# jdalcorso/radar-sounder-crw

Measured on AMD Instinct MI355X. Metric: radargram columns/sec (CRW fwd+bwd), higher is better.
Workload: dtype f32 (conv2-5 multiply on the bf16 matrix cores with hi/lo operand pairs, fp32 accumulate: fp32-grade; everything else fp32); 1 GPU; one synthetic 512x4096 radargram per GPU per step = 8 items [T=32,N=63,16x16] (patch 16x16, overlap (8, 0)), tau=0.01, CNN encoder, fwd+bwd+all-reduce+Adam; parallelism=dp1 (independent sequences), chain=fp32 MFMA 16x16x4, prefix form, encoder_convs=bf16x3

## Files before the change

radar-sounder-crw_amd/csrc/encoder_conv.hip:

```cpp
#include "crw_common.h"
#include <type_traits>
#include <cstdlib>

namespace crw {
namespace {

constexpr int IMG_W = 10, PAD_W = 12, NPIX = 100, NPAD = 144, MT = 7;

typedef __bf16 bf8 __attribute__((ext_vector_type(8)));
typedef short s4v __attribute__((ext_vector_type(4)));
typedef short s8v __attribute__((ext_vector_type(8)));
typedef __attribute__((address_space(3))) char *lds_cp;

__device__ inline uint16_t f2bf(float x) { return __builtin_bit_cast(uint16_t, (__bf16)x); }
__device__ inline float bf2f(uint16_t h) { return __builtin_bit_cast(float, (uint32_t)h << 16); }

template <int C>
constexpr int row_stride() { return C * 2 + 16; }
template <int C>
constexpr int plane_bytes() { return NPAD * row_stride<C>(); }
template <int C>
__device__ inline int px_off(int pp, int chunk) { return pp * row_stride<C>() + 16 * chunk; }
template <int C>
constexpr int crs() { return C * 2 + 32; }
// ... 485 lines not shown
  constexpr int NT = NCI / 16;
  constexpr int WCI = NT < 4 ? NT : 4, WCO = NW / WCI;
  constexpr int NCOW = NCO / 16 / WCO;
  static_assert(NT == WCI && COUT % NCO == 0 && CIN % NCI == 0, "tiling");
  constexpr int NGRP_CI = CIN / NCI;
  extern __shared__ __attribute__((aligned(16))) char lds[];
  char *xs = lds, *ys = lds + NPL * XPL;

  constexpr int NGRP = NGRP_CI * (COUT / NCO);
  const int wg_slice = a.xcd_map ? ((int)blockIdx.x / 8 / NGRP) * 8 + (int)blockIdx.x % 8 : (int)blockIdx.x / NGRP;
  const int wg_grp = a.xcd_map ? ((int)blockIdx.x / 8) % NGRP : (int)blockIdx.x % NGRP;
  const int grp_ci = wg_grp % NGRP_CI, grp_co = wg_grp / NGRP_CI;
  const int ci_base = grp_ci * NCI, co_base = grp_co * NCO;
  const int tid = threadIdx.x, lane = tid & 63, wave = tid >> 6, g = lane >> 4;
  const int wci = wave % WCI, wco = wave / WCI;
  const int co0w = wco * NCOW * 16;

  f32x4 acc[9][NCOW];
#pragma unroll
  for (int t = 0; t < 9; ++t)
#pragma unroll
    for (int j = 0; j < NCOW; ++j) acc[t][j] = f32x4{0.f, 0.f, 0.f, 0.f};
  f32x4 accb[NCOW];
#pragma unroll
  for (int j = 0; j < NCOW; ++j) accb[j] = f32x4{0.f, 0.f, 0.f, 0.f};
  const bool bias_wave = grp_ci == 0 && __builtin_amdgcn_readfirstlane(wci) == 0;

  const int p_begin = wg_slice * a.patches_per_block;
  const int p_end = min(a.P, p_begin + a.patches_per_block);
  const uint32_t xs_a = (uint32_t)(uintptr_t)(lds_cp)xs, ys_a = (uint32_t)(uintptr_t)(lds_cp)ys;

  for (int pl = 0; pl < NPL; ++pl) {
    zero_halo<NCI, NTH, XS>(xs + pl * XPL + XTAIL * XS, tid);
    for (int c = tid; c < XTAIL * XS / 16; c += NTH) *reinterpret_cast<uint4 *>(xs + pl * XPL + 16 * c) = uint4{0, 0, 0, 0};
    for (int c = tid; c < (1 + TAILPIX) * YS / 16; c += NTH) *reinterpret_cast<uint4 *>(ys + pl * YPL + NPIX * YS + 16 * c) = uint4{0, 0, 0, 0};
  }

  constexpr int XCH = NCI / 8, XTOT = NPIX * XCH, XIT = (XTOT + NTH - 1) / NTH;
  constexpr int YCH = NCO / 8, YTOT = NPIX * YCH, YIT = (YTOT + NTH - 1) / NTH;
  constexpr int TXC = XTAIL * XCH, TYC = TAILPIX * YCH, TTOT = NPL * (TXC + TYC), TIT = (TTOT + NTH - 1) / NTH;
#ifdef CRW_CONV_STAMPS
  long long ph_[4] = {0, 0, 0, 0}, prev_ = (long long)__builtin_amdgcn_s_memtime();
#define WG_STAMP(k) { const long long n_ = (long long)__builtin_amdgcn_s_memtime(); ph_[k] += n_ - prev_; prev_ = n_; }
#else
#define WG_STAMP(k)
#endif

  auto tail_src_dst = [&](int c, int &src, int &dst) {
    const int pl = c / (TXC + TYC), r = c % (TXC + TYC);
    if (r < TXC) {
      const int s = r / XCH, ch = r % XCH;
      dst = pl * XPL + s * XS + 16 * ch;
      src = pl * XPL + (XTAIL + 9 * PAD_W + s) * XS + 16 * ch;
    } else {
      const int q = r - TXC, j = q / YCH, ch = q % YCH;
      dst = NPL * XPL + pl * YPL + (YROWS + j) * YS + 16 * ch;
      src = NPL * XPL + pl * YPL + (NPIX - TAILPIX + j) * YS + 16 * ch;
    }
  };

  const int t16 = lane & 15, q4 = t16 >> 2, pq = t16 & 3;
  const uint32_t lane_col = 8 * (pq & 1) + 16 * (pq >> 1);
  auto row_addr = [&](int v, int carry, bool flush, uint32_t &ya, uint32_t &xa) {
    const int i = v - carry;
    int yrow = NPIX, xpix = XTAIL;
    if (v < carry) {
      const int t = NPIX - carry + v;
      yrow = YROWS + (t - (NPIX - TAILPIX));
      xpix = t - 90;
    } else if (!flush && i < NPIX) {
      yrow = i;
      xpix = XTAIL + (i / IMG_W) * PAD_W + (i % IMG_W);
    }
    ya = ys_a + yrow * YS + lane_col + 2 * co0w;
    xa = xs_a + xpix * XS + lane_col + 32 * wci;
  };
  auto kstep = [&](int ks, int carry, bool flush) {
    uint32_t ya_lo, ya_hi, xa_lo, xa_hi;
    row_addr(32 * ks + 4 * g + q4, carry, flush, ya_lo, xa_lo);
    row_addr(32 * ks + 4 * g + q4 + 16, carry, flush, ya_hi, xa_hi);
    bf8 ah[NCOW], al[NCOW];
    static_for<NCOW>([&](auto JC) {
      constexpr int j = decltype(JC)::value;
      ah[j] = tr_frag<32 * j>(ya_lo, ya_hi);
      if (SPLIT == 3) al[j] = tr_frag<YPL + 32 * j>(ya_lo, ya_hi);
    });
    bf8 bh[2], bl[2];
    auto read_b = [&](auto TC) {
      constexpr int tap = decltype(TC)::value;
      constexpr int XO = ((tap / 3) * PAD_W + (tap % 3)) * XS;
      bh[tap & 1] = tr_frag<XO>(xa_lo, xa_hi);
      if (SPLIT == 3) bl[tap & 1] = tr_frag<XPL + XO>(xa_lo, xa_hi);
    };
    read_b(std::integral_constant<int, 0>{});
    static_for<9>([&](auto TC) {
      constexpr int tap = decltype(TC)::value;
      if constexpr (tap < 8) {
        read_b(std::integral_constant<int, tap + 1>{});
        if (SPLIT == 3) asm volatile("s_waitcnt lgkmcnt(4)" ::: "memory");
        else asm volatile("s_waitcnt lgkmcnt(2)" ::: "memory");
      } else {
        asm volatile("s_waitcnt lgkmcnt(0)" ::: "memory");
      }
      __builtin_amdgcn_sched_barrier(0);
      if constexpr (tap == 0) {
        if (bias_wave) {
          const s8v o = {0x3f80, 0x3f80, 0x3f80, 0x3f80, 0x3f80, 0x3f80, 0x3f80, 0x3f80};
          const bf8 ones = __builtin_bit_cast(bf8, o);
#pragma unroll
          for (int j = 0; j < NCOW; ++j) {
            if (SPLIT == 3) accb[j] = __builtin_amdgcn_mfma_f32_16x16x32_bf16(al[j], ones, accb[j], 0, 0, 0);
            accb[j] = __builtin_amdgcn_mfma_f32_16x16x32_bf16(ah[j], ones, accb[j], 0, 0, 0);
          }
        }
      }
#pragma unroll
      for (int j = 0; j < NCOW; ++j) {
        if (SPLIT == 3) {
          acc[tap][j] = __builtin_amdgcn_mfma_f32_16x16x32_bf16(al[j], bh[tap & 1], acc[tap][j], 0, 0, 0);
          acc[tap][j] = __builtin_amdgcn_mfma_f32_16x16x32_bf16(ah[j], bl[tap & 1], acc[tap][j], 0, 0, 0);
        }
        acc[tap][j] = __builtin_amdgcn_mfma_f32_16x16x32_bf16(ah[j], bh[tap & 1], acc[tap][j], 0, 0, 0);
      }
    });
  };

  int carry = 0;
  uint4 tv[TIT];
#pragma unroll
  for (int i = 0; i < TIT; ++i) tv[i] = uint4{0, 0, 0, 0};
  if constexpr (MAP) {
    const int ntile = a.tiles_x * a.tiles_y;
    constexpr int WTOT = NPAD * XCH, WIT = (WTOT + NTH - 1) / NTH;
    for (int u = p_begin; u < p_end; ++u) {
      const int pq = u / ntile, tile = u % ntile;
      const int ty0 = (tile / a.tiles_x) * IMG_W, tx0 = (tile % a.tiles_x) * IMG_W;
      __syncthreads();
      for (int pl = 0; pl < NPL; ++pl) {
        uint4 xv[WIT];
        const uint16_t *src = (pl ? a.xl : a.xh) + ci_base;
#pragma unroll
        for (int i = 0; i < WIT; ++i) {
          const int c = min(tid + i * NTH, WTOT - 1), wp = c / XCH, ch = c % XCH;
          const int my = ty0 + wp / PAD_W - 1, mx = tx0 + wp % PAD_W - 1;
          const bool ok = my >= 0 && my < a.mh && mx >= 0 && mx < a.mw;
          const long off = (((long)pq * a.mh + min(max(my, 0), a.mh - 1)) * a.mw + min(max(mx, 0), a.mw - 1)) * CIN + 8 * ch;
          xv[i] = *reinterpret_cast<const uint4 *>(src + off);
          if (!ok) xv[i] = uint4{0, 0, 0, 0};
        }
#pragma unroll
        for (int i = 0; i < WIT; ++i) {
          const int c = tid + i * NTH;
          if (WTOT % NTH == 0 || c < WTOT) *reinterpret_cast<uint4 *>(xs + pl * XPL + (XTAIL + c / XCH) * XS + 16 * (c % XCH)) = xv[i];
        }
        uint4 yv[YIT];
        const uint16_t *ysrc = (pl ? a.dyl : a.dyh) + co_base;
#pragma unroll
        for (int i = 0; i < YIT; ++i) {
          const int c = min(tid + i * NTH, YTOT - 1), pix = c / YCH, ch = c % YCH;
          const int oy = ty0 + pix / IMG_W, ox = tx0 + pix % IMG_W;
          const bool ok = oy < a.mh && ox < a.mw;
          const long off = (((long)pq * a.mh + min(oy, a.mh - 1)) * a.mw + min(ox, a.mw - 1)) * COUT + 8 * ch;
          yv[i] = *reinterpret_cast<const uint4 *>(ysrc + off);
          if (!ok) yv[i] = uint4{0, 0, 0, 0};
        }
#pragma unroll
        for (int i = 0; i < YIT; ++i) {
          const int c = tid + i * NTH;
          if (YTOT % NTH == 0 || c < YTOT) *reinterpret_cast<uint4 *>(ys + pl * YPL + (c / YCH) * YS + 16 * (c % YCH)) = yv[i];
        }
      }
      __syncthreads();
#pragma unroll 1
      for (int ks = 0; ks < 4; ++ks) kstep(ks, 0, false);
    }
  }
  for (int p = MAP ? p_end : p_begin; p < p_end; ++p) {
    __syncthreads();
    WG_STAMP(3)
    {
#pragma unroll
      for (int i = 0; i < TIT; ++i) {
        const int c = tid + i * NTH;
        if (TTOT % NTH == 0 || c < TTOT) {
          int src, dst;
          tail_src_dst(c, src, dst);
          *reinterpret_cast<uint4 *>(xs + dst) = tv[i];
        }
      }
      uint4 xv[NPL][XIT], yv[NPL][YIT];
#pragma unroll
      for (int pl = 0; pl < NPL; ++pl) {
        const uint16_t *src = (pl ? a.xl : a.xh) + (long)p * NPIX * CIN + ci_base;
#pragma unroll
        for (int i = 0; i < XIT; ++i) {
          const int c = min(tid + i * NTH, XTOT - 1);
          xv[pl][i] = *reinterpret_cast<const uint4 *>(src + (long)(c / XCH) * CIN + 8 * (c % XCH));
        }
      }
#pragma unroll
      for (int pl = 0; pl < NPL; ++pl) {
        const uint16_t *src = ((pl && !a.dgap) ? a.dyl : a.dyh) + (long)p * NPIX * COUT + co_base;
#pragma unroll
        for (int i = 0; i < YIT; ++i) {
          const int c = min(tid + i * NTH, YTOT - 1);
          yv[pl][i] = *reinterpret_cast<const uint4 *>(src + (long)(c / YCH) * COUT + 8 * (c % YCH));
        }
      }
#pragma unroll
      for (int pl = 0; pl < NPL; ++pl)
#pragma unroll
        for (int i = 0; i < XIT; ++i) {
          const int c = tid + i * NTH;
          if (XTOT % NTH == 0 || c < XTOT)
            *reinterpret_cast<uint4 *>(xs + pl * XPL + (XTAIL + interior_pp(c / XCH)) * XS + 16 * (c % XCH)) = xv[pl][i];
        }
      if (a.dgap) {
        static_assert(NTH % YCH == 0, "a thread keeps its channel chunk");
        const int ch = tid % YCH;
        uint32_t gh[4], gl[4];
        gap_split8(a.dgap + (long)p * COUT + co_base + 8 * ch, gh, gl);
#pragma unroll
        for (int i = 0; i < YIT; ++i) {
          const int c = tid + i * NTH;
          if (YTOT % NTH == 0 || c < YTOT) {
            uint4 oh, ol;
            gap_mask8(yv[0][i], gh, gl, oh, ol);
            const int off = (c / YCH) * YS + 16 * ch;
            *reinterpret_cast<uint4 *>(ys + off) = oh;
            if (SPLIT == 3) *reinterpret_cast<uint4 *>(ys + YPL + off) = ol;
          }
        }
      } else {
#pragma unroll
        for (int pl = 0; pl < NPL; ++pl)
#pragma unroll
          for (int i = 0; i < YIT; ++i) {
            const int c = tid + i * NTH;
            if (YTOT % NTH == 0 || c < YTOT) *reinterpret_cast<uint4 *>(ys + pl * YPL + (c / YCH) * YS + 16 * (c % YCH)) = yv[pl][i];
          }
      }
    }
    __syncthreads();
    WG_STAMP(0)
    WG_STAMP(1)
#ifdef CRW_CONV_STAMPS
    if (a.stamps && tid == 0 && p - p_begin < 60)
      a.stamps[(long)blockIdx.x * 64 + 4 + (p - p_begin)] = (long long)__builtin_amdgcn_s_memtime();
#endif
    const int nks = carry == 8 ? 4 : 3;
#pragma unroll 1
    for (int ks = 0; ks < nks; ++ks) kstep(ks, carry, false);
    carry = carry == 8 ? 0 : carry + 4;
#pragma unroll
    for (int i = 0; i < TIT; ++i) {
      const int c = min(tid + i * NTH, TTOT - 1);
      int src, dst;
      tail_src_dst(c, src, dst);
      tv[i] = *reinterpret_cast<const uint4 *>(xs + src);
    }
    WG_STAMP(2)
  }
  if (carry > 0) {
    __syncthreads();
#pragma unroll
    for (int i = 0; i < TIT; ++i) {
      const int c = tid + i * NTH;
      if (TTOT % NTH == 0 || c < TTOT) {
        int src, dst;
        tail_src_dst(c, src, dst);
        *reinterpret_cast<uint4 *>(xs + dst) = tv[i];
      }
    }
    __syncthreads();
    kstep(0, carry, true);
  }
#ifdef CRW_CONV_STAMPS
  if (a.stamps && tid == 0)
    for (int k = 0; k < 4; ++k) a.stamps[(long)blockIdx.x * 64 + k] = ph_[k];
#endif

  float *dwp = a.dw_part + (long)wg_slice * COUT * CIN * 9;
#pragma unroll
  for (int tap = 0; tap < 9; ++tap)
#pragma unroll
    for (int j = 0; j < NCOW; ++j)
#pragma unroll
      for (int r = 0; r < 4; ++r) {
        const int co = co_base + co0w + 16 * j + 4 * g + r, ci = ci_base + 16 * wci + (lane & 15);
        dwp[((long)tap * COUT + co) * CIN + ci] = acc[tap][j][r];
      }
  if (bias_wave && (lane & 15) == 0) {
#pragma unroll
    for (int j = 0; j < NCOW; ++j)
#pragma unroll
      for (int r = 0; r < 4; ++r) a.db_part[(long)wg_slice * COUT + co_base + co0w + 16 * j + 4 * g + r] = accb[j][r];
  }
}

constexpr int W2_NCO = 128, W2_NCI = 64, W2_NW = 8, W2_KROWS = 32;
template <int C>
constexpr int w2_stride() { return 2 * C + 32; }

template <int SPLIT, int CIN, int COUT, int DIAG = 0>
__global__ __launch_bounds__(W2_NW * 64, 2) void conv3x3_wgrad2_kernel(WgradArgs a) {
  constexpr int NCO = W2_NCO, NCI = W2_NCI, NTH = W2_NW * 64, NPL = (SPLIT == 3) ? 2 : 1;
  constexpr int XS = w2_stride<NCI>(), XPL = NPAD * XS, XSLOT = NPL * XPL;
  constexpr int YS = w2_stride<NCO>(), YPL = W2_KROWS * YS, YSLOT = NPL * YPL;
  constexpr int NCOW = 4, WCI = 4;
  static_assert(COUT == NCO && CIN % NCI == 0, "tiling");
  constexpr int NGRP = CIN / NCI;
  extern __shared__ __attribute__((aligned(16))) char lds[];
  char *xs = lds, *ys = lds + 2 * XSLOT;
  char *gs = ys + 2 * YSLOT;

  const int wg_slice = a.xcd_map ? ((int)blockIdx.x / 8 / NGRP) * 8 + (int)blockIdx.x % 8 : (int)blockIdx.x / NGRP;
  const int grp_ci = a.xcd_map ? ((int)blockIdx.x / 8) % NGRP : (int)blockIdx.x % NGRP;
  const int ci_base = grp_ci * NCI;
  const int tid = threadIdx.x, lane = tid & 63, wave = tid >> 6, g = lane >> 4;
  const int wci = wave % WCI, wco = wave / WCI;
  const int wci_s = __builtin_amdgcn_readfirstlane(wci);
  const int co0w = wco * NCOW * 16;

  const int p_begin = wg_slice * a.patches_per_block;
  const int np = min(a.P, p_begin + a.patches_per_block) - p_begin;
  const int npx = np * NPIX;
  const int NK = (npx + W2_KROWS - 1) / W2_KROWS;

  f32x4 acc[9][NCOW];
#pragma unroll
  for (int t = 0; t < 9; ++t)
#pragma unroll
    for (int j = 0; j < NCOW; ++j) acc[t][j] = f32x4{0.f, 0.f, 0.f, 0.f};
  f32x4 accb = f32x4{0.f, 0.f, 0.f, 0.f};
  const bool bias_wg = grp_ci == 0;

  for (int c = tid; c < 2 * XSLOT / 16; c += NTH) *reinterpret_cast<uint4 *>(xs + 16 * c) = uint4{0, 0, 0, 0};

  const int yrow = tid >> 4, ych = tid & 15;
  constexpr int XCH = NCI / 8, XTOT = NPIX * XCH;
  typedef uint32_t u4v __attribute__((ext_vector_type(4)));
  const long dy_off = (long)p_begin * NPIX * COUT, x_off = (long)p_begin * NPIX * CIN + ci_base;
  const __amdgpu_buffer_rsrc_t dyh_rs = __builtin_amdgcn_make_buffer_rsrc((void *)(a.dyh + dy_off), 0, npx * COUT * 2, 0x00020000);
  const __amdgpu_buffer_rsrc_t dyl_rs = __builtin_amdgcn_make_buffer_rsrc(
      (void *)((SPLIT == 3 && !a.dgap ? a.dyl : a.dyh) + dy_off), 0, npx * COUT * 2, 0x00020000);
  const __amdgpu_buffer_rsrc_t xh_rs = __builtin_amdgcn_make_buffer_rsrc((void *)(a.xh + x_off), 0, (npx * CIN - ci_base) * 2, 0x00020000);
  const __amdgpu_buffer_rsrc_t xl_rs = __builtin_amdgcn_make_buffer_rsrc((void *)((SPLIT == 3 ? a.xl : a.xh) + x_off), 0,
                                                                          (npx * CIN - ci_base) * 2, 0x00020000);
  const int y_voff = (yrow * COUT + 8 * ych) * 2;
  int x_voff[2];
#pragma unroll
  for (int i = 0; i < 2; ++i) {
    const int c = min(tid + i * NTH, XTOT - 1);
    x_voff[i] = ((c / XCH) * CIN + 8 * (c % XCH)) * 2;
  }
  uint4 sy[NPL], sx[2];
  auto load_dy = [&](int n) {
    const int soff = n * (W2_KROWS * COUT * 2);
    constexpr int AUX = DIAG == 6 ? 2 : 0;
    sy[0] = __builtin_bit_cast(uint4, (u4v)__builtin_amdgcn_raw_buffer_load_b128(dyh_rs, y_voff, soff, AUX));
    if (SPLIT == 3 && !a.dgap) sy[NPL - 1] = __builtin_bit_cast(uint4, (u4v)__builtin_amdgcn_raw_buffer_load_b128(dyl_rs, y_voff, soff, AUX));
  };
  auto store_dy = [&](int n) {
    uint4 vh = sy[0], vl = uint4{0, 0, 0, 0};
    if (SPLIT == 3 && !a.dgap) vl = sy[NPL - 1];
    if (a.dgap) {
      const int q = (32 * n + yrow) / NPIX;
      const uint4 h4 = *reinterpret_cast<const uint4 *>(gs + (q & 1) * (4 * COUT) + 16 * ych);
      const uint4 l4 = *reinterpret_cast<const uint4 *>(gs + (q & 1) * (4 * COUT) + 2 * COUT + 16 * ych);
      const uint32_t gh[4] = {h4.x, h4.y, h4.z, h4.w}, gl[4] = {l4.x, l4.y, l4.z, l4.w};
      gap_mask8(sy[0], gh, gl, vh, vl);
    }
    char *dst = ys + (n & 1) * YSLOT + yrow * YS + 16 * ych;
    *reinterpret_cast<uint4 *>(dst) = vh;
    if (SPLIT == 3) *reinterpret_cast<uint4 *>(dst + YPL) = vl;
  };
  auto load_x = [&](int q, int pl) {
    const int soff = q * (NPIX * CIN * 2);
#pragma unroll
    for (int i = 0; i < 2; ++i)
      sx[i] = __builtin_bit_cast(uint4, (u4v)__builtin_amdgcn_raw_buffer_load_b128(pl ? xl_rs : xh_rs, x_voff[i], soff, DIAG == 6 ? 2 : 0));
  };
  auto store_x = [&](int q, int pl) {
    char *dst = xs + (q & 1) * XSLOT + pl * XPL;
#pragma unroll
    for (int i = 0; i < 2; ++i) {
      const int c = tid + i * NTH;
      if (c < XTOT) *reinterpret_cast<uint4 *>(dst + interior_pp(c / XCH) * XS + 16 * (c % XCH)) = sx[i];
    }
  };
  auto stage_gap = [&](int q) {
    if (tid < COUT / 8) {
      uint32_t gh[4], gl[4];
      gap_split8(a.dgap + (long)(p_begin + q) * COUT + 8 * tid, gh, gl);
      *reinterpret_cast<uint4 *>(gs + (q & 1) * (4 * COUT) + 16 * tid) = uint4{gh[0], gh[1], gh[2], gh[3]};
      *reinterpret_cast<uint4 *>(gs + (q & 1) * (4 * COUT) + 2 * COUT + 16 * tid) = uint4{gl[0], gl[1], gl[2], gl[3]};
    }
  };
  auto first_k = [&](int q) { return (q * NPIX) / W2_KROWS; };
  auto patch_starting_at = [&](int n) {
    if (n >= NK) return -1;
    const int q = min((32 * n + 31) / NPIX, np - 1);
    return first_k(q) == n ? q : -1;
  };

  const uint32_t xs_a = (uint32_t)(uintptr_t)(lds_cp)xs, ys_a = (uint32_t)(uintptr_t)(lds_cp)ys;
  const int t16 = lane & 15, q4 = t16 >> 2, pq = t16 & 3;
  const uint32_t lane_col = 8 * (pq & 1) + 16 * (pq >> 1);
  const int r_lo = 4 * g + q4, r_hi = r_lo + 16;
  const uint32_t ya_lo0 = ys_a + r_lo * YS + lane_col + 2 * co0w, ya_hi0 = ys_a + r_hi * YS + lane_col + 2 * co0w;
  auto x_addr = [&](int G) {
    const int Gc = min(G, npx - 1);
    const int q = Gc / NPIX, i = Gc - q * NPIX;
    return xs_a + (q & 1) * XSLOT + ((i / IMG_W) * PAD_W + (i % IMG_W)) * XS + lane_col + 32 * wci;
  };

  auto kstep = [&](int n) {
    const uint32_t ya_lo = ya_lo0 + (n & 1) * YSLOT, ya_hi = ya_hi0 + (n & 1) * YSLOT;
    const uint32_t xa_lo = x_addr(32 * n + r_lo), xa_hi = x_addr(32 * n + r_hi);
    bf8 ah[NCOW], al[NCOW];
    static_for<NCOW>([&](auto JC) {
      constexpr int j = decltype(JC)::value;
      ah[j] = tr_frag<32 * j>(ya_lo, ya_hi);
      if (SPLIT == 3) al[j] = tr_frag<YPL + 32 * j>(ya_lo, ya_hi);
    });
    bf8 bh[2], bl[2];
    auto read_b = [&](auto TC) {
      constexpr int tap = decltype(TC)::value;
      constexpr int XO = ((tap / 3) * PAD_W + (tap % 3)) * XS;
      bh[tap & 1] = tr_frag<XO>(xa_lo, xa_hi);
      if (SPLIT == 3) bl[tap & 1] = tr_frag<XPL + XO>(xa_lo, xa_hi);
    };
    read_b(std::integral_constant<int, 0>{});
    static_for<9>([&](auto TC) {
      constexpr int tap = decltype(TC)::value;
      if constexpr (tap < 8) {
        read_b(std::integral_constant<int, tap + 1>{});
        if (SPLIT == 3) asm volatile("s_waitcnt lgkmcnt(4)" ::: "memory");
        else asm volatile("s_waitcnt lgkmcnt(2)" ::: "memory");
      } else {
        asm volatile("s_waitcnt lgkmcnt(0)" ::: "memory");
      }
      __builtin_amdgcn_sched_barrier(0);
      if constexpr (tap == 0) {
        if (bias_wg) {
          const s8v o = {0x3f80, 0x3f80, 0x3f80, 0x3f80, 0x3f80, 0x3f80, 0x3f80, 0x3f80};
          const bf8 ones = __builtin_bit_cast(bf8, o);
          static_for<NCOW>([&](auto JC) {
            constexpr int j = decltype(JC)::value;
            if (wci_s == j) {
              if (SPLIT == 3) accb = __builtin_amdgcn_mfma_f32_16x16x32_bf16(al[j], ones, accb, 0, 0, 0);
              accb = __builtin_amdgcn_mfma_f32_16x16x32_bf16(ah[j], ones, accb, 0, 0, 0);
            }
          });
        }
      }
#pragma unroll
      for (int j = 0; j < NCOW; ++j) {
        if (SPLIT == 3) {
          acc[tap][j] = __builtin_amdgcn_mfma_f32_16x16x32_bf16(al[j], bh[tap & 1], acc[tap][j], 0, 0, 0);
          acc[tap][j] = __builtin_amdgcn_mfma_f32_16x16x32_bf16(ah[j], bl[tap & 1], acc[tap][j], 0, 0, 0);
        }
        acc[tap][j] = __builtin_amdgcn_mfma_f32_16x16x32_bf16(ah[j], bh[tap & 1], acc[tap][j], 0, 0, 0);
      }
    });
  };

  load_dy(0);
  load_x(0, 0);
  if (a.dgap) stage_gap(0);
  __syncthreads();
  store_x(0, 0);
  if (SPLIT == 3) {
    load_x(0, 1);
    store_x(0, 1);
  }
  store_dy(0);
  __syncthreads();

#pragma unroll 1
  for (int n = 0; n < NK; ++n) {
    const bool more = n + 1 < NK;
    const int q_2 = patch_starting_at(n + 2);
    const int q_hi = (SPLIT == 3) ? q_2 : -1;
    const int q_lo = patch_starting_at(n + 1);
    const int xq = q_lo >= 0 ? q_lo : q_hi, xpl = q_lo >= 0 ? NPL - 1 : 0;
    if (DIAG != 2 && DIAG != 3 && DIAG != 5) {
      load_dy(more ? n + 1 : n);
      load_x(xq >= 0 ? xq : 0, xpl);
    }
    kstep(n);
    if (DIAG == 2 || DIAG == 3) {
      if (DIAG & 1) continue;
      __syncthreads();
      continue;
    }
    if (DIAG == 4) {
      asm volatile("" ::"v"(sy[0].x), "v"(sy[NPL - 1].y), "v"(sx[0].x), "v"(sx[1].y));
      __syncthreads();
      continue;
    }
    if (more) store_dy(n + 1);
    if (xq >= 0) store_x(xq, xpl);
    if (a.dgap && q_2 >= 0) stage_gap(q_2);
    if (!(DIAG & 1)) __syncthreads();
  }

  float *dwp = a.dw_part + (long)wg_slice * COUT * CIN * 9;
#pragma unroll
  for (int tap = 0; tap < 9; ++tap)
#pragma unroll
    for (int j = 0; j < NCOW; ++j)
#pragma unroll
      for (int r = 0; r < 4; ++r) {
        const int co = co0w + 16 * j + 4 * g + r, ci = ci_base + 16 * wci + (lane & 15);
        dwp[((long)tap * COUT + co) * CIN + ci] = acc[tap][j][r];
      }
  if (bias_wg && (lane & 15) == 0) {
#pragma unroll
    for (int r = 0; r < 4; ++r) a.db_part[(long)wg_slice * COUT + co0w + 16 * wci + 4 * g + r] = accb[r];
  }
}

__global__ __launch_bounds__(256) void slice_sum_kernel(const float *__restrict__ part, int nslice, long n,
                                                        float *__restrict__ out) {
  for (long e = (long)blockIdx.x * 256 + threadIdx.x; e < n; e += (long)gridDim.x * 256) {
    float s = 0.f;
    for (int k = 0; k < nslice; ++k) s += part[(long)k * n + e];
    out[e] = s;
  }
}

__global__ __launch_bounds__(256) void slice_sum_dw_kernel(const float *__restrict__ part, int nslice, int coci,
                                                           float *__restrict__ out, int nblk_dw,
                                                           const float *__restrict__ bpart, int cout, float *__restrict__ bout) {
  __shared__ float red[4][64];
  const long n = 9L * coci;
  const int lane = threadIdx.x & 63, q = threadIdx.x >> 6;
  if ((int)blockIdx.x >= nblk_dw) {
    const int e = ((int)blockIdx.x - nblk_dw) * 4 + q;
    if (e >= cout) return;
    float s = 0.f;
    for (int k = lane; k < nslice; k += 64) s += bpart[(long)k * cout + e];
    s = wave_sum(s);
    if (lane == 0) bout[e] = s;
    return;
  }
  const long e = (long)blockIdx.x * 64 + lane;
  const int per = (nslice + 3) / 4, k0 = q * per, k1 = min(nslice, k0 + per);
  float s = 0.f;
  if (e < n) {
    int k = k0;
    for (; k + 8 <= k1; k += 8) {
      float v[8];
#pragma unroll
      for (int u = 0; u < 8; ++u) v[u] = part[(long)(k + u) * n + e];
#pragma unroll
      for (int u = 0; u < 8; ++u) s += v[u];
    }
    for (; k < k1; ++k) s += part[(long)k * n + e];
  }
  red[q][lane] = s;
  __syncthreads();
  if (q == 0 && e < n) {
    const float t = (red[0][lane] + red[1][lane]) + (red[2][lane] + red[3][lane]);
    const int tap = e / coci, cc = e % coci;
    out[(long)cc * 9 + tap] = t;
  }
}

__device__ inline long frag_index(int tap, int n, int k, int N, int K) {
  return ((((long)tap * (K / 32) + k / 32) * (N / 16) + n / 16) * 64 + ((k % 32) / 8) * 16 + n % 16) * 8 + k % 8;
}
__global__ __launch_bounds__(256) void pack_weights_kernel(const float *__restrict__ w, int CO, int CI,
                                                           uint16_t *fh, uint16_t *fl, uint16_t *bh, uint16_t *bl) {
  const long n = (long)CO * CI * 9;
  for (long e = (long)blockIdx.x * 256 + threadIdx.x; e < n; e += (long)gridDim.x * 256) {
    const int tap = e % 9, ci = (e / 9) % CI, co = e / (9L * CI);
    const float v = w[e];
    const uint16_t h = f2bf(v), l = f2bf(v - bf2f(h));
    const long of = frag_index(tap, co, ci, CO, CI), ob = frag_index(8 - tap, ci, co, CI, CO);
    fh[of] = h; bh[ob] = h;
    if (fl) { fl[of] = l; bl[ob] = l; }
  }
}

__global__ __launch_bounds__(256) void pack_input_kernel(const float *__restrict__ x, int P, int C, int npix, uint16_t *xh,
                                                         uint16_t *xl) {
  const long n = (long)P * npix * C;
  for (long e = (long)blockIdx.x * 256 + threadIdx.x; e < n; e += (long)gridDim.x * 256) {
    const int c = e % C, i = (e / C) % npix;
    const long p = e / ((long)C * npix);
    const float v = x[(p * C + c) * npix + i];
    const uint16_t h = f2bf(v);
    xh[e] = h;
    if (xl) xl[e] = f2bf(v - bf2f(h));
  }
}

__global__ __launch_bounds__(256) void gap_bwd_kernel(const float *__restrict__ dgap, const uint16_t *__restrict__ yh,
                                                      int P, int C, int npix, uint16_t *dh, uint16_t *dl) {
  const long n8 = (long)P * npix * C / 8;
  const int c8 = C / 8;
  const float inv = 1.0f / (float)npix;
  for (long e = (long)blockIdx.x * 256 + threadIdx.x; e < n8; e += (long)gridDim.x * 256) {
#pragma clang fp contract(off)
    const int c = (int)(e % c8) * 8;
    const long p = e / ((long)c8 * npix);
    const uint4 y = *reinterpret_cast<const uint4 *>(yh + e * 8);
    const float4 g0 = *reinterpret_cast<const float4 *>(dgap + p * C + c), g1 = *reinterpret_cast<const float4 *>(dgap + p * C + c + 4);
    const float gv[8] = {g0.x, g0.y, g0.z, g0.w, g1.x, g1.y, g1.z, g1.w};
    const uint32_t yw[4] = {y.x, y.y, y.z, y.w};
    uint32_t h[4], l[4];
#pragma unroll
    for (int w = 0; w < 4; ++w) {
      const float a0 = (yw[w] & 0x7fffu) ? gv[2 * w] * inv : 0.f, a1 = (yw[w] & 0x7fff0000u) ? gv[2 * w + 1] * inv : 0.f;
      const uint16_t h0 = f2bf(a0), h1 = f2bf(a1);
      h[w] = (uint32_t)h0 | ((uint32_t)h1 << 16);
      l[w] = (uint32_t)f2bf(a0 - bf2f(h0)) | ((uint32_t)f2bf(a1 - bf2f(h1)) << 16);
    }
    *reinterpret_cast<uint4 *>(dh + e * 8) = uint4{h[0], h[1], h[2], h[3]};
    if (dl) *reinterpret_cast<uint4 *>(dl + e * 8) = uint4{l[0], l[1], l[2], l[3]};
  }
}

template <int C>
constexpr size_t conv_lds_bytes(int npl) { return (size_t)(npl - 1) * PLANE_ROWS * crs<C>() + (size_t)NPAD * crs<C>(); }

template <int SPLIT, int CIN, int COUT, int MODE, int NW>
int launch_conv_nw(const ConvArgs &a, hipStream_t s) {
  constexpr int CMAX = CIN > COUT ? CIN : COUT;
  size_t lds = conv_lds_bytes<CMAX>(SPLIT == 3 ? 2 : 1);
#ifdef CRW_CONV_STAMPS
  if (const char *e = getenv("CRW_CONV_LDS_PAD")) lds += (size_t)atoi(e);
#endif
  static bool attr = false;
  if (!attr && lds > 64 * 1024) {
    if (hipFuncSetAttribute((const void *)conv3x3_kernel<SPLIT, CIN, COUT, MODE, NW>,
                            hipFuncAttributeMaxDynamicSharedMemorySize, (int)lds) != hipSuccess) {
      g_last_hip_error = (int)hipGetLastError();
      return CRW_EHIP;
    }
    attr = true;
  }
  hipLaunchKernelGGL((conv3x3_kernel<SPLIT, CIN, COUT, MODE, NW>), dim3(a.P), dim3(NW * 64), lds, s, a);
  return check_launch();
}

constexpr int MT_SMALL = 4;

template <int SPLIT, int CIN, int COUT, int MODE, int MTL>
int launch_conv_map_cls(const ConvArgs &a, hipStream_t s) {
  constexpr int CMAX = CIN > COUT ? CIN : COUT, NW = (SPLIT == 3 ? 8 : 4);
  const size_t lds = (size_t)(SPLIT == 3 ? 2 : 1) * NPAD * row_stride<CMAX>();
  static bool attr = false;
  if (!attr && lds > 64 * 1024) {
    if (hipFuncSetAttribute((const void *)conv3x3_kernel<SPLIT, CIN, COUT, MODE, NW, true, MTL>,
                            hipFuncAttributeMaxDynamicSharedMemorySize, (int)lds) != hipSuccess) {
      g_last_hip_error = (int)hipGetLastError();
      return CRW_EHIP;
    }
    attr = true;
  }
  hipLaunchKernelGGL((conv3x3_kernel<SPLIT, CIN, COUT, MODE, NW, true, MTL>), dim3(a.P * a.ncls), dim3(NW * 64), lds, s, a);
  return check_launch();
}

template <int SPLIT, int CIN, int COUT, int MODE = 0>
int launch_conv_map(const ConvArgs &a0, hipStream_t s) {
  const int ntile = a0.tiles_x * a0.tiles_y;
  if (ntile > 65535) return CRW_EINVAL;
  constexpr int CHUNK = (int)(sizeof(a0.tile_list) / sizeof(a0.tile_list[0]));
  ConvArgs big = a0, small = a0;
  big.ncls = small.ncls = 0;
  for (int t = 0; t < ntile; ++t) {
    const int th = std::min(IMG_W, a0.mh - (t / a0.tiles_x) * IMG_W), tw = std::min(IMG_W, a0.mw - (t % a0.tiles_x) * IMG_W);
    if (tw * th > 16 * MT_SMALL) {
      big.tile_list[big.ncls++] = (unsigned short)t;
      if (big.ncls == CHUNK) {
        CRW_TRY((launch_conv_map_cls<SPLIT, CIN, COUT, MODE, MT>(big, s)));
        big.ncls = 0;
      }
    } else {
      small.tile_list[small.ncls++] = (unsigned short)t;
      if (small.ncls == CHUNK) {
        CRW_TRY((launch_conv_map_cls<SPLIT, CIN, COUT, MODE, MT_SMALL>(small, s)));
        small.ncls = 0;
      }
    }
  }
  if (big.ncls) CRW_TRY((launch_conv_map_cls<SPLIT, CIN, COUT, MODE, MT>(big, s)));
  if (small.ncls) CRW_TRY((launch_conv_map_cls<SPLIT, CIN, COUT, MODE, MT_SMALL>(small, s)));
  return CRW_OK;
}

template <int SPLIT, int CIN, int COUT, int MODE>
int launch_conv(const ConvArgs &a, hipStream_t s) {
  static const char *force = getenv("CRW_CONV_NW");
  if (force && force[0] == '4') return launch_conv_nw<SPLIT, CIN, COUT, MODE, 4>(a, s);
  if (force && force[0] == '8') return launch_conv_nw<SPLIT, CIN, COUT, MODE, 8>(a, s);
  return launch_conv_nw<SPLIT, CIN, COUT, MODE, (SPLIT == 3 ? 8 : 4)>(a, s);
}

constexpr int wgrad_nci(int cin) { return cin > 64 ? 64 : cin; }

template <int SPLIT, int CIN, int COUT>
int launch_wgrad(const WgradArgs &a, int nblk, hipStream_t s) {
  constexpr int NCI = wgrad_nci(CIN), NW = SPLIT == 3 ? 4 : 8;
  const size_t lds = (size_t)(SPLIT == 3 ? 2 : 1) * ((XTAIL + NPAD) * row_stride<NCI>() + YROWS_ALL * row_stride<WG_NCO>());
  static bool attr = false;
  if (!attr && lds > 64 * 1024) {
    if (hipFuncSetAttribute((const void *)conv3x3_wgrad_kernel<SPLIT, CIN, COUT, NCI, NW>,
                            hipFuncAttributeMaxDynamicSharedMemorySize, (int)lds) != hipSuccess) {
      g_last_hip_error = (int)hipGetLastError();
      return CRW_EHIP;
    }
    attr = true;
  }
  hipLaunchKernelGGL((conv3x3_wgrad_kernel<SPLIT, CIN, COUT, NCI, NW>), dim3(nblk * (CIN / NCI) * (COUT / WG_NCO)),
                     dim3(NW * 64), lds, s, a);
  return check_launch();
}

template <int SPLIT, int CIN, int COUT>
int launch_wgrad_map(const WgradArgs &a, int nblk, hipStream_t s) {
  constexpr int NCI = wgrad_nci(CIN), NW = SPLIT == 3 ? 4 : 8;
  const size_t lds = (size_t)(SPLIT == 3 ? 2 : 1) * ((XTAIL + NPAD) * row_stride<NCI>() + YROWS_ALL * row_stride<WG_NCO>());
  static bool attr = false;
  if (!attr && lds > 64 * 1024) {
    if (hipFuncSetAttribute((const void *)conv3x3_wgrad_kernel<SPLIT, CIN, COUT, NCI, NW, true>,
                            hipFuncAttributeMaxDynamicSharedMemorySize, (int)lds) != hipSuccess) {
      g_last_hip_error = (int)hipGetLastError();
      return CRW_EHIP;
    }
    attr = true;
  }
  hipLaunchKernelGGL((conv3x3_wgrad_kernel<SPLIT, CIN, COUT, NCI, NW, true>), dim3(nblk * (CIN / NCI) * (COUT / WG_NCO)),
                     dim3(NW * 64), lds, s, a);
  return check_launch();
}

template <int SPLIT, int CIN, int COUT, int DIAG = 0>
int launch_wgrad2(const WgradArgs &a, int nslice, hipStream_t s) {
  constexpr int NPL = SPLIT == 3 ? 2 : 1;
  const size_t lds = (size_t)2 * NPL * (NPAD * w2_stride<W2_NCI>() + W2_KROWS * w2_stride<W2_NCO>()) + 2 * 4 * W2_NCO;
  static bool attr = false;
  if (!attr) {
    if (hipFuncSetAttribute((const void *)conv3x3_wgrad2_kernel<SPLIT, CIN, COUT, DIAG>, hipFuncAttributeMaxDynamicSharedMemorySize,
                            (int)lds) != hipSuccess) {
      g_last_hip_error = (int)hipGetLastError();
      return CRW_EHIP;
    }
    attr = true;
  }
  hipLaunchKernelGGL((conv3x3_wgrad2_kernel<SPLIT, CIN, COUT, DIAG>), dim3(nslice * (CIN / W2_NCI)), dim3(W2_NW * 64), lds, s, a);
  return check_launch();
}

inline int ew_grid(long n) {
  long b = (n + 255) / 256;
  return (int)(b > 8192 ? 8192 : (b < 1 ? 1 : b));
}

}
}

using namespace crw;

long long *g_conv_stamps = nullptr;

extern "C" {

#ifdef CRW_CONV_STAMPS
void crw_debug_conv_stamps(long long *buf) { g_conv_stamps = buf; }
#endif

int crw_enc_pack_weights(const float *w, int cout, int cin, uint16_t *fwd_hi, uint16_t *fwd_lo, uint16_t *bwd_hi,
                         uint16_t *bwd_lo, crw_stream_t stream) {
  clear_stale_error();
  if (!w || !fwd_hi || !bwd_hi || cout < 1 || cin < 1 || (fwd_lo == nullptr) != (bwd_lo == nullptr)) return CRW_EINVAL;
  hipLaunchKernelGGL(pack_weights_kernel, dim3(ew_grid((long)cout * cin * 9)), dim3(256), 0, (hipStream_t)stream, w, cout,
                     cin, fwd_hi, fwd_lo, bwd_hi, bwd_lo);
  return check_launch();
}

int crw_enc_pack_input(const float *x, int P, int C, uint16_t *xh, uint16_t *xl, crw_stream_t stream) {
  clear_stale_error();
  if (!x || !xh || P < 1 || C < 8 || C % 8) return CRW_EINVAL;
  hipLaunchKernelGGL(pack_input_kernel, dim3(ew_grid((long)P * NPIX * C)), dim3(256), 0, (hipStream_t)stream, x, P, C,
                     NPIX, xh, xl);
  return check_launch();
}

int crw_enc_pack_input_map(const float *x, int P, int C, int H, int W, uint16_t *xh, uint16_t *xl, crw_stream_t stream) {
  clear_stale_error();
  if (!x || !xh || P < 1 || C < 8 || C % 8 || H < 1 || W < 1) return CRW_EINVAL;
  hipLaunchKernelGGL(pack_input_kernel, dim3(ew_grid((long)P * H * W * C)), dim3(256), 0, (hipStream_t)stream, x, P, C,
                     H * W, xh, xl);
  return check_launch();
}

int crw_enc_conv3x3_map(int mode, int split, int P, int H, int W, int cin, int cout, const uint16_t *x_hi, const uint16_t *x_lo,
                        const uint16_t *w_hi, const uint16_t *w_lo, const float *bias, const uint16_t *mask_hi, uint16_t *y_hi,
                        uint16_t *y_lo, float *y_f32, float *gap_part, crw_stream_t stream) {
  clear_stale_error();
  if (!x_hi || !w_hi || P < 1 || H < 1 || W < 1 || (split != 1 && split != 3) || (mode != 0 && mode != 1)) return CRW_EINVAL;
  if (split == 3 && (!w_lo || !x_lo)) return CRW_EINVAL;
  if (!y_hi && !gap_part && !y_f32) return CRW_EINVAL;
  if (mode == 1 && (gap_part || bias)) return CRW_EINVAL;
  const int tx = (W + IMG_W - 1) / IMG_W, ty = (H + IMG_W - 1) / IMG_W;
  if ((long)P * tx * ty > 0x7fffffffL) return CRW_EINVAL;
  ConvArgs a{x_hi, x_lo, w_hi, w_lo, bias, mask_hi, y_hi, y_lo, y_f32, gap_part, nullptr, P, nullptr, H, W, tx, ty, 0, {}};
  hipStream_t s = (hipStream_t)stream;
#define CRW_MAP_CASE(CI, CO, MODE) \
  if (mode == MODE && cin == CI && cout == CO) return split == 3 ? launch_conv_map<3, CI, CO, MODE>(a, s) : launch_conv_map<1, CI, CO, MODE>(a, s);
  CRW_MAP_CASE(32, 64, 0)
  CRW_MAP_CASE(64, 128, 0)
  CRW_MAP_CASE(128, 128, 0)
  CRW_MAP_CASE(128, 128, 1)
  CRW_MAP_CASE(128, 64, 1)
  CRW_MAP_CASE(64, 32, 1)
#undef CRW_MAP_CASE
  return CRW_EINVAL;
}

int crw_enc_gap_bwd(const float *dgap, const uint16_t *y_hi, int P, int C, int npix, uint16_t *dy_hi, uint16_t *dy_lo,
                    crw_stream_t stream) {
  clear_stale_error();
  if (!dgap || !y_hi || !dy_hi || P < 1 || C < 8 || C % 8 || npix < 1) return CRW_EINVAL;
  hipLaunchKernelGGL(gap_bwd_kernel, dim3(ew_grid((long)P * npix * C / 8)), dim3(256), 0, (hipStream_t)stream, dgap, y_hi, P,
                     C, npix, dy_hi, dy_lo);
  return check_launch();
}

int crw_enc_conv3x3(int mode, int split, int P, int cin, int cout, const uint16_t *x_hi, const uint16_t *x_lo,
                    const uint16_t *w_hi, const uint16_t *w_lo, const float *bias, const uint16_t *mask_hi,
                    uint16_t *y_hi, uint16_t *y_lo, float *y_f32, float *gap, const float *dgap, crw_stream_t stream) {
  clear_stale_error();
  if (!x_hi || !w_hi || P < 1 || (mode != 0 && mode != 1) || (split != 1 && split != 3)) return CRW_EINVAL;
  if (split == 3 && (!w_lo || (!x_lo && !dgap))) return CRW_EINVAL;
  if (dgap && mode != 1) return CRW_EINVAL;
  if (!y_hi && !y_f32 && !gap) return CRW_EINVAL;
  ConvArgs a{x_hi, x_lo, w_hi, w_lo, bias, mask_hi, y_hi, y_lo, y_f32, gap, dgap, P, g_conv_stamps, 0, 0, 1, 1};
  hipStream_t s = (hipStream_t)stream;
#define CRW_CONV_CASE(CI, CO)                                                                      \
  if (cin == CI && cout == CO) {                                                                   \
    if (split == 3) return mode == 0 ? launch_conv<3, CI, CO, 0>(a, s) : launch_conv<3, CI, CO, 1>(a, s); \
    return mode == 0 ? launch_conv<1, CI, CO, 0>(a, s) : launch_conv<1, CI, CO, 1>(a, s);           \
  }
  CRW_CONV_CASE(32, 64)
  CRW_CONV_CASE(64, 128)
  CRW_CONV_CASE(128, 128)
  CRW_CONV_CASE(128, 64)
  CRW_CONV_CASE(64, 32)
#undef CRW_CONV_CASE
  return CRW_EINVAL;
}

static int wgrad_groups(int cin) { return cin / wgrad_nci(cin); }

static int wgrad_slices(int P, int cin, int cout, int split) {
  (void)split;
  const int groups = wgrad_groups(cin) * (cout / WG_NCO);
  int n = 256 * 2 / (groups < 1 ? 1 : groups);
  return n > P ? P : n;
}

size_t crw_enc_wgrad_ws_bytes(int P, int cin, int cout, int split) {
  if (P < 1 || cin < 1 || cout < 1) return 0;
  return (size_t)wgrad_slices(P, cin, cout, split) *
         ((size_t)cout * cin * 9 + (size_t)wgrad_groups(cin) * cout) * sizeof(float);
}

int crw_enc_conv3x3_wgrad(int split, int P, int cin, int cout, const uint16_t *dy_hi, const uint16_t *dy_lo,
                          const uint16_t *x_hi, const uint16_t *x_lo, const float *dgap, float *dw, float *db, void *ws,
                          size_t ws_bytes, crw_stream_t stream) {
  clear_stale_error();
  if (!dy_hi || !x_hi || !dw || !db || !ws || P < 1 || (split != 1 && split != 3)) return CRW_EINVAL;
  if (split == 3 && ((!dy_lo && !dgap) || !x_lo)) return CRW_EINVAL;
  if (ws_bytes < crw_enc_wgrad_ws_bytes(P, cin, cout, split)) return CRW_EWORKSPACE;
  hipStream_t s = (hipStream_t)stream;
  int nslice = wgrad_slices(P, cin, cout, split);
  static const char *force = getenv("CRW_WGRAD");
  const bool streamed = cout == W2_NCO && cin % W2_NCI == 0 && !(force && force[0] == '1');
  if (streamed) {
    const int n2 = 256 / (cin / W2_NCI);
    nslice = n2 > P ? P : n2;
  }
  int ppb = (P + nslice - 1) / nslice;
  if (streamed) nslice = (P + ppb - 1) / ppb;
  float *dw_part = static_cast<float *>(ws), *db_part = dw_part + (size_t)nslice * cout * cin * 9;
  WgradArgs a{dy_hi, dy_lo, x_hi, x_lo, dgap, dw_part, db_part, P, ppb, nslice % 8 == 0 ? 1 : 0, g_conv_stamps, 0, 0, 1, 1};
  int st = CRW_EINVAL;
  if (streamed) {
    if (cin == 64) st = split == 3 ? launch_wgrad2<3, 64, 128>(a, nslice, s) : launch_wgrad2<1, 64, 128>(a, nslice, s);
    else if (cin == 128) {
#ifdef CRW_CONV_STAMPS
      static const char *diag = getenv("CRW_WGRAD_DIAG");
      if (diag && split == 3 && diag[0] == '1') return launch_wgrad2<3, 128, 128, 1>(a, nslice, s);
      if (diag && split == 3 && diag[0] == '2') return launch_wgrad2<3, 128, 128, 2>(a, nslice, s);
      if (diag && split == 3 && diag[0] == '3') return launch_wgrad2<3, 128, 128, 3>(a, nslice, s);
      if (diag && split == 3 && diag[0] == '4') return launch_wgrad2<3, 128, 128, 4>(a, nslice, s);
      if (diag && split == 3 && diag[0] == '5') return launch_wgrad2<3, 128, 128, 5>(a, nslice, s);
      if (diag && split == 3 && diag[0] == '6') return launch_wgrad2<3, 128, 128, 6>(a, nslice, s);
#endif
      st = split == 3 ? launch_wgrad2<3, 128, 128>(a, nslice, s) : launch_wgrad2<1, 128, 128>(a, nslice, s);
    }
  } else {
#define CRW_WG_CASE(CI, CO)                                                                  \
  if (cin == CI && cout == CO) st = split == 3 ? launch_wgrad<3, CI, CO>(a, nslice, s) : launch_wgrad<1, CI, CO>(a, nslice, s);
  CRW_WG_CASE(32, 64)
  CRW_WG_CASE(64, 128)
  CRW_WG_CASE(128, 128)
#undef CRW_WG_CASE
  }
  if (st != CRW_OK) return st;
  const long nw = (long)cout * cin * 9;
  const int nblk_dw = (int)((nw + 63) / 64);
  hipLaunchKernelGGL(slice_sum_dw_kernel, dim3((unsigned)(nblk_dw + (cout + 3) / 4)), dim3(256), 0, s, dw_part, nslice, cout * cin,
                     dw, nblk_dw, db_part, cout, db);
  return check_launch();
}


int crw_enc_conv3x3_wgrad_map(int split, int P, int H, int W, int cin, int cout, const uint16_t *dy_hi, const uint16_t *dy_lo,
                              const uint16_t *x_hi, const uint16_t *x_lo, float *dw, float *db, void *ws, size_t ws_bytes,
                              crw_stream_t stream) {
  clear_stale_error();
  if (!dy_hi || !x_hi || !dw || !db || !ws || P < 1 || H < 1 || W < 1 || (split != 1 && split != 3)) return CRW_EINVAL;
  if (split == 3 && (!dy_lo || !x_lo)) return CRW_EINVAL;
  const int tx = (W + IMG_W - 1) / IMG_W, ty = (H + IMG_W - 1) / IMG_W;
  const long units_l = (long)P * tx * ty;
  if (units_l > 0x7fffffffL) return CRW_EINVAL;
  const int units = (int)units_l;
  if (ws_bytes < crw_enc_wgrad_ws_bytes(units, cin, cout, split)) return CRW_EWORKSPACE;
  hipStream_t s = (hipStream_t)stream;
  int nslice = wgrad_slices(units, cin, cout, split);
  const int upb = (units + nslice - 1) / nslice;
  nslice = (units + upb - 1) / upb;
  float *dw_part = static_cast<float *>(ws), *db_part = dw_part + (size_t)nslice * cout * cin * 9;
  WgradArgs a{dy_hi, dy_lo, x_hi, x_lo, nullptr, dw_part, db_part, units, upb, nslice % 8 == 0 ? 1 : 0, nullptr, H, W, tx, ty};
  int st = CRW_EINVAL;
#define CRW_WGM_CASE(CI, CO) \
  if (cin == CI && cout == CO) st = split == 3 ? launch_wgrad_map<3, CI, CO>(a, nslice, s) : launch_wgrad_map<1, CI, CO>(a, nslice, s);
  CRW_WGM_CASE(32, 64)
  CRW_WGM_CASE(64, 128)
  CRW_WGM_CASE(128, 128)
#undef CRW_WGM_CASE
  if (st != CRW_OK) return st;
  const long nw = (long)cout * cin * 9;
  const int nblk_dw = (int)((nw + 63) / 64);
  hipLaunchKernelGGL(slice_sum_dw_kernel, dim3((unsigned)(nblk_dw + (cout + 3) / 4)), dim3(256), 0, s, dw_part, nslice, cout * cin,
                     dw, nblk_dw, db_part, cout, db);
  return check_launch();
}

}
```

Measured before the change: 641,100 radargram columns/s.

## Interleave LDS stores and next-address math into wgrad2 MFMA tap loop

Restructures the streamed weight-gradient kernel's k-step so the LDS staging stores for the next step, and the precomputed x addresses for that step, are issued in the middle of the 9-tap MFMA sequence instead of after it. For split=3, the B fragment for tap 0 is also read before the A fragments, and the tap-0 MFMAs are gated per-j with graded lgkmcnt waits so matrix work can start before all A reads land. Default forms are chosen per split via a FORM bitmask, and further variants are selectable through the diag environment variable. This aims to hide LDS write and address latency behind matrix-core work, at the cost of more scheduling barriers and more live registers.

```diff
diff --git a/radar-sounder-crw_amd/csrc/encoder_conv.hip b/radar-sounder-crw_amd/csrc/encoder_conv.hip
--- a/radar-sounder-crw_amd/csrc/encoder_conv.hip
+++ b/radar-sounder-crw_amd/csrc/encoder_conv.hip
@@ -811,8 +811,12 @@
 template <int C>
 constexpr int w2_stride() { return 2 * C + 32; }
 
-template <int SPLIT, int CIN, int COUT, int DIAG = 0>
+constexpr int w2_form(int split) { return split == 3 ? (1 | 2 | 4 | (1 << 3)) : (1 | (3 << 3)); }
+template <int SPLIT, int CIN, int COUT, int DIAG_ = 0>
 __global__ __launch_bounds__(W2_NW * 64, 2) void conv3x3_wgrad2_kernel(WgradArgs a) {
+  constexpr int DIAG = DIAG_ >= 16 ? 0 : DIAG_, FORM = DIAG_ >= 16 ? DIAG_ - 16 : w2_form(SPLIT);
+  constexpr bool MID = FORM & 1, PREADDR = FORM & 2, ORDERED = FORM & 4;
+  constexpr int TS = 4 + ((FORM >> 3) & 3);
   constexpr int NCO = W2_NCO, NCI = W2_NCI, NTH = W2_NW * 64, NPL = (SPLIT == 3) ? 2 : 1;
   constexpr int XS = w2_stride<NCI>(), XPL = NPAD * XS, XSLOT = NPL * XPL;
   constexpr int YS = w2_stride<NCO>(), YPL = W2_KROWS * YS, YSLOT = NPL * YPL;
@@ -865,7 +869,7 @@
   }
   uint4 sy[NPL], sx[2];
   auto load_dy = [&](int n) {
-    const int soff = n * (W2_KROWS * COUT * 2);
+    const int soff = __builtin_amdgcn_readfirstlane(n) * (W2_KROWS * COUT * 2);
     constexpr int AUX = DIAG == 6 ? 2 : 0;
     sy[0] = __builtin_bit_cast(uint4, (u4v)__builtin_amdgcn_raw_buffer_load_b128(dyh_rs, y_voff, soff, AUX));
     if (SPLIT == 3 && !a.dgap) sy[NPL - 1] = __builtin_bit_cast(uint4, (u4v)__builtin_amdgcn_raw_buffer_load_b128(dyl_rs, y_voff, soff, AUX));
@@ -924,33 +928,66 @@
     return xs_a + (q & 1) * XSLOT + ((i / IMG_W) * PAD_W + (i % IMG_W)) * XS + lane_col + 32 * wci;
   };
 
-  auto kstep = [&](int n) {
+  auto kstep = [&](int n, uint32_t xa_lo, uint32_t xa_hi, auto &&mid) {
     const uint32_t ya_lo = ya_lo0 + (n & 1) * YSLOT, ya_hi = ya_hi0 + (n & 1) * YSLOT;
-    const uint32_t xa_lo = x_addr(32 * n + r_lo), xa_hi = x_addr(32 * n + r_hi);
     bf8 ah[NCOW], al[NCOW];
-    static_for<NCOW>([&](auto JC) {
-      constexpr int j = decltype(JC)::value;
-      ah[j] = tr_frag<32 * j>(ya_lo, ya_hi);
-      if (SPLIT == 3) al[j] = tr_frag<YPL + 32 * j>(ya_lo, ya_hi);
-    });
     bf8 bh[2], bl[2];
+    auto read_a = [&] {
+      static_for<NCOW>([&](auto JC) {
+        constexpr int j = decltype(JC)::value;
+        ah[j] = tr_frag<32 * j>(ya_lo, ya_hi);
+        if (SPLIT == 3) al[j] = tr_frag<YPL + 32 * j>(ya_lo, ya_hi);
+      });
+    };
     auto read_b = [&](auto TC) {
       constexpr int tap = decltype(TC)::value;
       constexpr int XO = ((tap / 3) * PAD_W + (tap % 3)) * XS;
       bh[tap & 1] = tr_frag<XO>(xa_lo, xa_hi);
       if (SPLIT == 3) bl[tap & 1] = tr_frag<XPL + XO>(xa_lo, xa_hi);
     };
-    read_b(std::integral_constant<int, 0>{});
+    constexpr int RD = 2 * NPL;
+    if (ORDERED) {
+      read_b(std::integral_constant<int, 0>{});
+      read_a();
+    } else {
+      read_a();
+      read_b(std::integral_constant<int, 0>{});
+    }
     static_for<9>([&](auto TC) {
       constexpr int tap = decltype(TC)::value;
+      if constexpr (MID && tap == TS + 1) __builtin_amdgcn_sched_barrier(0);
       if constexpr (tap < 8) {
         read_b(std::integral_constant<int, tap + 1>{});
-        if (SPLIT == 3) asm volatile("s_waitcnt lgkmcnt(4)" ::: "memory");
-        else asm volatile("s_waitcnt lgkmcnt(2)" ::: "memory");
+        if constexpr (!(ORDERED && tap == 0)) asm volatile("s_waitcnt lgkmcnt(%0)" ::"n"(RD) : "memory");
       } else {
         asm volatile("s_waitcnt lgkmcnt(0)" ::: "memory");
       }
       __builtin_amdgcn_sched_barrier(0);
+      if constexpr (MID && tap == TS) {
+        mid();
+        __builtin_amdgcn_sched_barrier(0);
+      }
+      if constexpr (ORDERED && tap == 0) {
+        static_for<NCOW>([&](auto JC) {
+          constexpr int j = decltype(JC)::value;
+          constexpr int CNT = (4 - j) * RD > 15 ? 15 : (4 - j) * RD;
+          asm volatile("s_waitcnt lgkmcnt(%0)" ::"n"(CNT) : "memory");
+          __builtin_amdgcn_sched_barrier(0);
+          if (bias_wg && wci_s == j) {
+            const s8v o = {0x3f80, 0x3f80, 0x3f80, 0x3f80, 0x3f80, 0x3f80, 0x3f80, 0x3f80};
+            const bf8 ones = __builtin_bit_cast(bf8, o);
+            if (SPLIT == 3) accb = __builtin_amdgcn_mfma_f32_16x16x32_bf16(al[j], ones, accb, 0, 0, 0);
+            accb = __builtin_amdgcn_mfma_f32_16x16x32_bf16(ah[j], ones, accb, 0, 0, 0);
+          }
+          if (SPLIT == 3) {
+            acc[0][j] = __builtin_amdgcn_mfma_f32_16x16x32_bf16(al[j], bh[0], acc[0][j], 0, 0, 0);
+            acc[0][j] = __builtin_amdgcn_mfma_f32_16x16x32_bf16(ah[j], bl[0], acc[0][j], 0, 0, 0);
+          }
+          acc[0][j] = __builtin_amdgcn_mfma_f32_16x16x32_bf16(ah[j], bh[0], acc[0][j], 0, 0, 0);
+          __builtin_amdgcn_sched_barrier(0);
+        });
+        return;
+      }
       if constexpr (tap == 0) {
         if (bias_wg) {
           const s8v o = {0x3f80, 0x3f80, 0x3f80, 0x3f80, 0x3f80, 0x3f80, 0x3f80, 0x3f80};
@@ -987,6 +1024,7 @@
   store_dy(0);
   __syncthreads();
 
+  uint32_t xa_lo = x_addr(r_lo), xa_hi = x_addr(r_hi);
 #pragma unroll 1
   for (int n = 0; n < NK; ++n) {
     const bool more = n + 1 < NK;
@@ -998,20 +1036,37 @@
       load_dy(more ? n + 1 : n);
       load_x(xq >= 0 ? xq : 0, xpl);
     }
-    kstep(n);
-    if (DIAG == 2 || DIAG == 3) {
-      if (DIAG & 1) continue;
-      __syncthreads();
-      continue;
-    }
-    if (DIAG == 4) {
-      asm volatile("" ::"v"(sy[0].x), "v"(sy[NPL - 1].y), "v"(sx[0].x), "v"(sx[1].y));
-      __syncthreads();
-      continue;
-    }
-    if (more) store_dy(n + 1);
-    if (xq >= 0) store_x(xq, xpl);
-    if (a.dgap && q_2 >= 0) stage_gap(q_2);
+    auto stores = [&] {
+      if (DIAG == 2 || DIAG == 3) return;
+      if (DIAG == 4) {
+        asm volatile("" ::"v"(sy[0].x), "v"(sy[NPL - 1].y), "v"(sx[0].x), "v"(sx[1].y));
+        return;
+      }
+      if (more) store_dy(n + 1);
+      if (xq >= 0) store_x(xq, xpl);
+      if (a.dgap && q_2 >= 0) stage_gap(q_2);
+    };
+    uint32_t nxa_lo = 0, nxa_hi = 0;
+    auto next_addr = [&] {
+      nxa_lo = x_addr(32 * (n + 1) + r_lo);
+      nxa_hi = x_addr(32 * (n + 1) + r_hi);
+    };
+    if (!PREADDR) {
+      xa_lo = x_addr(32 * n + r_lo);
+      xa_hi = x_addr(32 * n + r_hi);
+    }
+    kstep(n, xa_lo, xa_hi, [&] {
+      stores();
+      if (PREADDR) next_addr();
+    });
+    if (!MID) {
+      stores();
+      if (PREADDR) next_addr();
+    }
+    if (PREADDR) {
+      xa_lo = nxa_lo;
+      xa_hi = nxa_hi;
+    }
     if (!(DIAG & 1)) __syncthreads();
   }
 
@@ -1406,12 +1461,20 @@
     else if (cin == 128) {
 #ifdef CRW_CONV_STAMPS
       static const char *diag = getenv("CRW_WGRAD_DIAG");
-      if (diag && split == 3 && diag[0] == '1') return launch_wgrad2<3, 128, 128, 1>(a, nslice, s);
-      if (diag && split == 3 && diag[0] == '2') return launch_wgrad2<3, 128, 128, 2>(a, nslice, s);
-      if (diag && split == 3 && diag[0] == '3') return launch_wgrad2<3, 128, 128, 3>(a, nslice, s);
-      if (diag && split == 3 && diag[0] == '4') return launch_wgrad2<3, 128, 128, 4>(a, nslice, s);
-      if (diag && split == 3 && diag[0] == '5') return launch_wgrad2<3, 128, 128, 5>(a, nslice, s);
-      if (diag && split == 3 && diag[0] == '6') return launch_wgrad2<3, 128, 128, 6>(a, nslice, s);
+      const int dv = diag ? atoi(diag) : 0;
+#define CRW_W2_DIAG(D) \
+  if (dv == D && split == 3) return launch_wgrad2<3, 128, 128, D>(a, nslice, s);
+      CRW_W2_DIAG(1) CRW_W2_DIAG(2) CRW_W2_DIAG(3) CRW_W2_DIAG(4) CRW_W2_DIAG(5) CRW_W2_DIAG(6)
+#undef CRW_W2_DIAG
+#define CRW_W2_FORM(F) \
+  if (dv == 16 + (F)) st = split == 3 ? launch_wgrad2<3, 128, 128, 16 + (F)>(a, nslice, s) : launch_wgrad2<1, 128, 128, 16 + (F)>(a, nslice, s);
+      CRW_W2_FORM(0)
+      CRW_W2_FORM(1) CRW_W2_FORM(9) CRW_W2_FORM(17) CRW_W2_FORM(25)
+      CRW_W2_FORM(2) CRW_W2_FORM(4)
+      CRW_W2_FORM(7) CRW_W2_FORM(15) CRW_W2_FORM(23) CRW_W2_FORM(31)
+      CRW_W2_FORM(6) CRW_W2_FORM(13) CRW_W2_FORM(11)
+#undef CRW_W2_FORM
+      if (dv < 16)
 #endif
       st = split == 3 ? launch_wgrad2<3, 128, 128>(a, nslice, s) : launch_wgrad2<1, 128, 128>(a, nslice, s);
     }
```

Result: no change. 642,000 radargram columns/s (median of 4 runs) (+0.1%).
